# wonheeML/mtl-ssl

Hardware: AMD Instinct MI355X
Metric: images/sec training, Faster R-CNN ResNet-101 + aux heads (higher is better)
Workload: dtype f32; 1 GPU; Faster R-CNN ResNet-101 + window/closeness/edgemask heads + refine, synthetic 1024x600 COCO-shaped (90 classes), per-GPU batch 2 (BASELINE.json configs[1]); global_batch=2, parallelism=dp1, pipeline_config=configs/frcnn_resnet101_coco_mtl.config

## Files before the change

include/mtlssl_hip.h:

```cpp
#ifndef MTLSSL_HIP_H_
#define MTLSSL_HIP_H_

#include <stdint.h>

#ifdef __cplusplus
extern "C" {
#endif

typedef void* mtlssl_stream_t;

#define MTLSSL_OK 0
#define MTLSSL_EINVAL (-1)
#define MTLSSL_ELAUNCH (-2)
#define MTLSSL_ECOMM (-3)

#define MTLSSL_ABI_VERSION 12

const char* mtlssl_last_error(void);
int mtlssl_abi_version(void);

int mtlssl_exp_rn(const double* x, double* y, int64_t n, mtlssl_stream_t stream);

typedef struct {
  int32_t N, H, W, C;
  int32_t K, R, S;
  int32_t OH, OW;
  int32_t stride, dilation;
  int32_t pad_t, pad_l;
  int32_t ldy;
} mtlssl_conv_desc;

#define MTLSSL_EPI_BIAS 1
#define MTLSSL_EPI_RESIDUAL 2
#define MTLSSL_EPI_RELU 4
#define MTLSSL_EPI_TANH 8
#define MTLSSL_EPI_RELU6 16
#define MTLSSL_EPI_MASK 32
#define MTLSSL_EPI_ACCUM 64
#define MTLSSL_EPI_MASK6 128

int64_t mtlssl_conv2d_workspace_bytes(const mtlssl_conv_desc* d, int mode);
int mtlssl_conv2d_fwd(const mtlssl_conv_desc* d, const float* x, const float* w,
                      const float* bias, const float* residual, float* y, int epilogue,
                      void* workspace, mtlssl_stream_t stream);
int mtlssl_conv2d_dgrad(const mtlssl_conv_desc* d, const float* dy, const float* w,
                        const float* residual, const float* mask_ref, float* dx, int epilogue,
                        void* workspace, mtlssl_stream_t stream);
int64_t mtlssl_conv2d_filter_xf_bytes(const mtlssl_conv_desc* d, int mode);
int mtlssl_conv2d_filter_xf_variant(const mtlssl_conv_desc* d, int mode);
int mtlssl_conv2d_transform_filter(const mtlssl_conv_desc* d, int mode, int variant, const float* w, float* filter_xf,
                                   mtlssl_stream_t stream);
int mtlssl_conv2d_transform_filters(int variant, int n, const void* w_ptrs, const void* xf_ptrs, const int64_t* ck,
                                    const int32_t* flip, int64_t max_ck, mtlssl_stream_t stream);
int mtlssl_conv2d_fwd_xf(const mtlssl_conv_desc* d, const float* x, const float* w, const float* bias,
                         const float* residual, float* y, int epilogue, void* workspace, const float* filter_xf,
                         int xf_variant, mtlssl_stream_t stream);
int mtlssl_conv2d_dgrad_xf(const mtlssl_conv_desc* d, const float* dy, const float* w, const float* residual,
                           const float* mask_ref, float* dx, int epilogue, void* workspace, const float* filter_xf,
                           int xf_variant, mtlssl_stream_t stream);
int64_t mtlssl_conv2d_input_xf_bytes(const mtlssl_conv_desc* d, int variant);
int mtlssl_conv2d_fwd_keep(const mtlssl_conv_desc* d, const float* x, const float* w, const float* bias,
                           const float* residual, float* y, int epilogue, void* workspace, const float* filter_xf,
                           int xf_variant, float* input_xf, int input_variant, mtlssl_stream_t stream);
int mtlssl_conv2d_wgrad_xf(const mtlssl_conv_desc* d, const float* x, const float* dy,
                           const float* out_scale, float* dw, float* dbias, float beta,
                           void* workspace, const float* input_xf, int input_variant, mtlssl_stream_t stream);
#define MTLSSL_CONV_GROUP_MAX 4
typedef struct {
  const float* w;
// ... 114 lines not shown
#define MTLSSL_EVAL_NMS_STANDARD 1
#define MTLSSL_EVAL_NMS_SOFT_LINEAR 2
#define MTLSSL_EVAL_NMS_SOFT_GAUSSIAN 3
int mtlssl_eval_nms(const float* boxes, const float* scores, const int32_t* segment_offsets, int num_segments,
                    int max_segment, int nms_type, double iou_threshold, double sigma, double scale_y, double scale_x,
                    int max_output, int32_t* index_out, float* scores_out, int32_t* count_out,
                    mtlssl_stream_t stream);
int mtlssl_edgemask_agreement(const float* logits, int Hf, int Wf, const float* gt_mask, int h, int w,
                              int32_t* count_out, mtlssl_stream_t stream);

#define MTLSSL_AUX_MAX_GT 256
#define MTLSSL_AUX_WINDOW_ATTEMPTS 100
int mtlssl_aux_draw_windows(const float* boxes_norm, const int32_t* num, int batch, int max_gt, int num_windows,
                            double height, double width, double min_obj_size, uint32_t seed, uint32_t step,
                            uint32_t image0, float* window_boxes, mtlssl_stream_t stream);
int mtlssl_aux_window_labels(const float* boxes_norm, const float* classes_bg, const int32_t* num,
                             const float* window_boxes, int batch, int max_gt, int num_classes, int num_windows,
                             double height, double width, float* labels_out, mtlssl_stream_t stream);
int mtlssl_aux_closeness(const float* boxes_norm, const float* classes_bg, const int32_t* num, int batch, int max_gt,
                         int num_classes, double height, double width, float* closeness_out, mtlssl_stream_t stream);
int mtlssl_aux_edgemask(const float* boxes_norm, const int32_t* num, int batch, int max_gt, double height, double width,
                        int mask_size, float* edgemask_out, mtlssl_stream_t stream);

int64_t mtlssl_assign_targets_workspace_bytes(int batch, int n, int max_gt);
int mtlssl_assign_targets(const float* anchors, int anchors_batched, int batch, int n,
                          const float* gt_boxes, const int32_t* num_gt, int max_gt,
                          const float* gt_labels, int label_dim, const float* gt_extra,
                          int extra_dim, const float* unmatched_cls_target, float matched_thresh,
                          float unmatched_thresh, int force_match, int32_t* match_out,
                          float* cls_targets_out, float* cls_weights_out, float* reg_targets_out,
                          float* reg_weights_out, float* extra_targets_out, void* workspace,
                          mtlssl_stream_t stream);

int mtlssl_balanced_sample(const float* indicator, const float* labels, int batch, int n,
                           int batch_size, float positive_fraction, uint32_t seed,
                           uint32_t stream_id0, uint32_t stream_stride, float* sampled_out,
                           mtlssl_stream_t stream);

int mtlssl_sample_proposals(const float* proposals, const int32_t* num_proposals, int batch,
                            int max_p, const float* gt_boxes, const int32_t* num_gt, int max_gt,
                            const float* gt_labels_bg, int label_dim, int n2,
                            float balance_fraction, uint32_t seed, uint32_t stream_id0,
                            uint32_t stream_stride, float img_h, float img_w,
                            float* boxes_abs_out, float* boxes_norm_out, int32_t* num_out,
                            mtlssl_stream_t stream);

int mtlssl_roi_crop_pool_fwd(const float* feat, int B, int H, int W, int C, const float* boxes,
                             const int32_t* box_ind, int R, int crop, int pool_k, int pool_stride,
                             float* out, uint8_t* argmax_out, mtlssl_stream_t stream);
int mtlssl_roi_crop_pool_bwd(const float* dout, const uint8_t* argmax, int B, int H, int W, int C,
                             const float* boxes, const int32_t* box_ind, int R, int crop,
                             int pool_k, int pool_stride, float* dfeat, mtlssl_stream_t stream);
int64_t mtlssl_roi_crop_pool_bwd_workspace_bytes(void);
int mtlssl_roi_crop_pool_bwd_ex(const float* dout, const uint8_t* argmax, int B, int H, int W, int C,
                                const float* boxes, const int32_t* box_ind, int R, int crop, int pool_k,
                                int pool_stride, float* dfeat, int accumulate, int algo, void* workspace,
                                mtlssl_stream_t stream);

int mtlssl_psroi_fwd(const float* fmap, int B, int H, int W, int C, const float* boxes,
                     const int32_t* box_ind, int R, int crop_h, int crop_w, int bins_y, int bins_x,
                     float* out, mtlssl_stream_t stream);
int mtlssl_psroi_bwd(const float* dout, int B, int H, int W, int C, const float* boxes,
                     const int32_t* box_ind, int R, int crop_h, int crop_w, int bins_y, int bins_x,
                     float* dfmap, mtlssl_stream_t stream);

int mtlssl_resize_bilinear_fwd(const float* x, float* y, int N, int H, int W, int C, int OH,
                               int OW, mtlssl_stream_t stream);
int mtlssl_resize_bilinear_bwd(const float* dy, float* dx, int N, int H, int W, int C, int OH,
                               int OW, mtlssl_stream_t stream);

typedef struct {
  int64_t offset;
  int32_t H, W;
  int32_t flip;
  float sy, sx;
  int32_t pad;
} mtlssl_image_desc;
int mtlssl_prepare_images(const uint8_t* pixels, const mtlssl_image_desc* desc, int B, int OH, int OW, float* out,
                          mtlssl_stream_t stream);
int64_t mtlssl_prepare_images_aug_workspace(int B, int n_contrast, int max_H);
int mtlssl_prepare_images_aug(const uint8_t* pixels, const mtlssl_image_desc* desc, int B, int OH, int OW,
                              const int32_t* prog, int n_ops, const float* params, int P, int max_H, void* workspace,
                              int64_t workspace_bytes, float* out, mtlssl_stream_t stream);


int mtlssl_smooth_l1_fwd_bwd(const float* pred, const float* target, const float* row_scale,
                             int rows, int code_size, float sigma, float* row_loss_out,
                             float* dpred_out, mtlssl_stream_t stream);
int mtlssl_softmax_ce_fwd_bwd(const float* logits, int ld_logits, const float* targets,
                              int ld_targets, int col0, int C, const float* row_scale, int rows,
                              float* row_loss_out, float* dlogits_out, mtlssl_stream_t stream);
int mtlssl_reduce_sum(const float* x, int n, float scale, float* out, mtlssl_stream_t stream);

int64_t mtlssl_sgd_workspace_bytes(int num_vars, int64_t max_var_size);
int mtlssl_sgd_momentum_clip(float* weights, const float* grads, float* accum,
                             const int32_t* var_offsets, int num_vars, int64_t total,
                             int64_t max_var_size, float lr, float momentum, float clip_norm,
                             float grad_scale, const float* var_weight_decay, const float* var_grad_mult,
                             float* norms_ws, mtlssl_stream_t stream);
int mtlssl_sgd_momentum_clip_fold(float* weights, float* grads, float* accum,
                                  const int32_t* var_offsets, int num_vars, int64_t total,
                                  int64_t max_var_size, float lr, float momentum, float clip_norm,
                                  float grad_scale, const float* var_weight_decay, const float* var_grad_mult,
                                  float* norms_ws, float* eff, const void* scale_ptrs, const int32_t* scale_len,
                                  int zero_grads, mtlssl_stream_t stream);
int mtlssl_adaptive_update_clip(int kind, float* weights, const float* grads, float* slot0, float* slot1,
// ... 78 lines not shown
```

mtl_ssl_amd/csrc/ops.hip:

```cpp
#include "common.h"

namespace mtlssl {

struct CropGeom {
  float y1, x1, hs, ws;
  int b;
};
__device__ __forceinline__ CropGeom crop_geom(const float* boxes, const int32_t* box_ind, int r,
                                              int H, int W, int crop) {
  float4 bx = *reinterpret_cast<const float4*>(boxes + (int64_t)r * 4);
  CropGeom g;
  g.b = box_ind[r];
  if (crop > 1) {
    g.hs = (bx.z - bx.x) * (float)(H - 1) / (float)(crop - 1);
    g.ws = (bx.w - bx.y) * (float)(W - 1) / (float)(crop - 1);
    g.y1 = bx.x * (float)(H - 1);
    g.x1 = bx.y * (float)(W - 1);
  } else {
    g.hs = 0.f; g.ws = 0.f;
    g.y1 = 0.5f * (bx.x + bx.z) * (float)(H - 1);
    g.x1 = 0.5f * (bx.y + bx.w) * (float)(W - 1);
  }
  return g;
}
// ... 134 lines not shown
    int dy = s / pk, dx = s % pk;
    float in_y = g.y1 + (float)(py * ps + dy) * g.hs;
    float in_x = g.x1 + (float)(px * ps + dx) * g.ws;
    if (in_y < 0.f || in_y > (float)(H - 1) || in_x < 0.f || in_x > (float)(W - 1)) continue;
    int ty = (int)floorf(in_y), by = (int)ceilf(in_y);
    int lx = (int)floorf(in_x), rx = (int)ceilf(in_x);
    float yl = in_y - (float)ty, xl = in_x - (float)lx;
    float dtop = (1.f - yl) * gr, dbot = yl * gr;
    unsafeAtomicAdd(fb + ((int64_t)ty * W + lx) * C + c, (1.f - xl) * dtop);
    unsafeAtomicAdd(fb + ((int64_t)ty * W + rx) * C + c, xl * dtop);
    unsafeAtomicAdd(fb + ((int64_t)by * W + lx) * C + c, (1.f - xl) * dbot);
    unsafeAtomicAdd(fb + ((int64_t)by * W + rx) * C + c, xl * dbot);
  }
}

constexpr int kRoiSlice = 16;
constexpr int kRoiPass = 512;
constexpr int kRoiThreads = 512;
struct RoiItem { float y1, x1, hs, ws; };

__global__ void __launch_bounds__(256) k_absmax_bits(const float* __restrict__ x, int64_t n4, uint32_t* out) {
  uint32_t m = 0;
  const int64_t stride = (int64_t)gridDim.x * 256;
  const uint4* x4 = reinterpret_cast<const uint4*>(x);
  int64_t i = (int64_t)blockIdx.x * 256 + threadIdx.x;
  for (; i + 3 * stride < n4; i += 4 * stride) {
    uint4 a = x4[i], b = x4[i + stride], c = x4[i + 2 * stride], d = x4[i + 3 * stride];
    uint32_t ma = max(max(a.x & 0x7fffffffu, a.y & 0x7fffffffu), max(a.z & 0x7fffffffu, a.w & 0x7fffffffu));
    uint32_t mb = max(max(b.x & 0x7fffffffu, b.y & 0x7fffffffu), max(b.z & 0x7fffffffu, b.w & 0x7fffffffu));
    uint32_t mc = max(max(c.x & 0x7fffffffu, c.y & 0x7fffffffu), max(c.z & 0x7fffffffu, c.w & 0x7fffffffu));
    uint32_t md = max(max(d.x & 0x7fffffffu, d.y & 0x7fffffffu), max(d.z & 0x7fffffffu, d.w & 0x7fffffffu));
    m = max(m, max(max(ma, mb), max(mc, md)));
  }
  for (; i < n4; i += stride) {
    uint4 a = x4[i];
    m = max(m, max(max(a.x & 0x7fffffffu, a.y & 0x7fffffffu), max(a.z & 0x7fffffffu, a.w & 0x7fffffffu)));
  }
#pragma unroll
  for (int o = 32; o > 0; o >>= 1) m = max(m, (uint32_t)__shfl_xor((int)m, o, 64));
  __shared__ uint32_t s_m[4];
  if ((threadIdx.x & 63) == 0) s_m[threadIdx.x >> 6] = m;
  __syncthreads();
  if (threadIdx.x == 0) {
    m = max(max(s_m[0], s_m[1]), max(s_m[2], s_m[3]));
    if (m) atomicMax(out, m);
  }
}

template <int PK>
__global__ void __launch_bounds__(kRoiThreads)
    k_roi_crop_pool_bwd_lds(const float* __restrict__ dout, const uint8_t* __restrict__ argmax, int H,
                            int W, int C, const float* __restrict__ boxes,
                            const int32_t* __restrict__ box_ind, int R, int crop, int pk_rt, int ps, int PH,
                            int PW, int band_rows, int nbands, int accumulate,
                            const uint32_t* __restrict__ absmax_bits, float* __restrict__ dfeat) {
  extern __shared__ __attribute__((aligned(16))) unsigned char s_raw[];
  const int pk = PK ? PK : pk_rt;
  const int NP = band_rows * W;
  unsigned long long* acc = reinterpret_cast<unsigned long long*>(s_raw);
  RoiItem* s_geom = reinterpret_cast<RoiItem*>(acc + (size_t)kRoiSlice * NP);
  int* s_roi = reinterpret_cast<int*>(s_geom + kRoiPass);
  uint16_t* s_entry = reinterpret_cast<uint16_t*>(s_roi + kRoiPass);
  __shared__ int s_n;
  int nblk = gridDim.x, bid = blockIdx.x;
  if (nblk % 8 == 0) bid = (bid % 8) * (nblk / 8) + bid / 8;
  const int band = bid % nbands;
  const int slice = (bid / nbands) % (C / kRoiSlice);
  const int img = bid / nbands / (C / kRoiSlice);
  const int row0 = band * band_rows;
  const int rows = min(band_rows, H - row0);
  const int tid = threadIdx.x;
  const uint32_t mbits = *absmax_bits;
  const bool finite = mbits < 0x7f800000u;
  int e = (int)(mbits >> 23) - 126;
  e = max(e, -90);
  const float scale = __uint_as_float((uint32_t)(30 - e + 127) << 23);
  const double descale = __longlong_as_double((long long)(e - 30 + 1023) << 52);
  for (int i = tid; i < kRoiSlice * NP; i += kRoiThreads) acc[i] = 0ull;
  const int quad = tid & 3;
  const int cslot = tid >> 2;
  unsigned long long* qacc = acc + (size_t)(quad * 4) * NP;
  const float inv_pw = 1.0f / (float)PW;
  const int cells = PH * PW;
  const float Hm1 = (float)(H - 1), Wm1 = (float)(W - 1);
  for (int base = 0; base < R; base += kRoiPass) {
    if (tid == 0) s_n = 0;
    __syncthreads();
    int lim = min(R, base + kRoiPass);
    for (int r = base + tid; r < lim; r += kRoiThreads) {
      if (box_ind[r] != img) continue;
      CropGeom g = crop_geom(boxes, box_ind, r, H, W, crop);
      int lo = PH, hi = -1;
      for (int py = 0; py < PH; ++py) {
        float ya = g.y1 + (float)(py * ps) * g.hs, yb = g.y1 + (float)(py * ps + pk - 1) * g.hs;
        float mn = fminf(ya, yb), mx = fmaxf(ya, yb);
        if (floorf(mn) < (float)(row0 + rows) && ceilf(mx) >= (float)row0) { lo = min(lo, py); hi = max(hi, py); }
      }
      if (hi < lo) continue;
      int slot = r - base;
      s_geom[slot] = RoiItem{g.y1, g.x1, g.hs, g.ws};
      s_roi[slot] = r;
      int pos = atomicAdd(&s_n, hi - lo + 1);
      for (int py = lo; py <= hi; ++py) s_entry[pos + py - lo] = (uint16_t)(slot * 64 + py);
    }
    __syncthreads();
    const int ncell = s_n * PW;
    RoiItem g_n = {0.f, 0.f, 0.f, 0.f};
    float4 gr_n = make_float4(0.f, 0.f, 0.f, 0.f);
    uint32_t am_n = 0u;
    int py_n = 0, px_n = 0;
    bool ok_n = false;
    auto fetch = [&](int ci) {
      ok_n = ci < ncell;
      if (!ok_n) return;
      int ei = (int)(((float)ci + 0.5f) * inv_pw);
      px_n = ci - ei * PW;
      int ent = s_entry[ei];
      int slot = ent >> 6;
      py_n = ent & 63;
      g_n = s_geom[slot];
      int64_t o = ((int64_t)s_roi[slot] * cells + py_n * PW + px_n) * C + slice * kRoiSlice + quad * 4;
      gr_n = *reinterpret_cast<const float4*>(dout + o);
      am_n = argmax ? *reinterpret_cast<const uint32_t*>(argmax + o) : 0u;
    };
    fetch(cslot);
    for (int c0 = 0; c0 < ncell; c0 += kRoiThreads / 4) {
      const RoiItem g = g_n;
      const float4 gr4 = gr_n;
      const uint32_t am4 = am_n;
      const int py = py_n, px = px_n;
      const bool ok = ok_n;
      fetch(c0 + kRoiThreads / 4 + cslot);
      if (!ok) continue;
      float grv[4] = {gr4.x, gr4.y, gr4.z, gr4.w};
      if (PK == 1) {
        float in_y = g.y1 + (float)(py * ps) * g.hs, in_x = g.x1 + (float)(px * ps) * g.ws;
        if (in_y < 0.f || in_y > Hm1 || in_x < 0.f || in_x > Wm1) continue;
        int ty = (int)floorf(in_y), by = (int)ceilf(in_y), lx = (int)floorf(in_x), rx = (int)ceilf(in_x);
        float yl = in_y - (float)ty, xl = in_x - (float)lx;
        int t = ty - row0, b = by - row0;
        bool okt = t >= 0 && t < rows, okb = b >= 0 && b < rows;
// ... 964 lines not shown
    o[e] *= sc[r];
    r = r + 1 == K ? 0 : r + 1;
  }
  *reinterpret_cast<float4*>(eff + i) = make_float4(o[0], o[1], o[2], o[3]);
}
__global__ void k_tanh_bwd(const float* y, const float* dy, float* dx, int64_t n) {
  int64_t i = blockIdx.x * (int64_t)blockDim.x + threadIdx.x;
  if (i < n) dx[i] = dy[i] * (1.f - y[i] * y[i]);
}

}

using namespace mtlssl;

extern "C" {

int mtlssl_roi_crop_pool_fwd(const float* feat, int B, int H, int W, int C, const float* boxes,
                             const int32_t* box_ind, int R, int crop, int pk, int ps, float* out,
                             uint8_t* argmax, mtlssl_stream_t stream) {
  MTLSSL_REQUIRE(C % 4 == 0, "roi_crop: C must be a multiple of 4");
  MTLSSL_REQUIRE(pk >= 1 && ps >= 1 && crop >= pk && pk * pk <= 255, "roi_crop: bad pool geometry");
  if (R == 0) return MTLSSL_OK;
  int PH = (crop - pk) / ps + 1;
  const char* algo = getenv("MTLSSL_ROI_FWD");
  if (C % 32 == 0 && C / 32 <= 256 && pk <= 2 && algo && !strcmp(algo, "xcd")) {
    const char* se = getenv("MTLSSL_ROI_SLICES");
    int nsl = se ? atoi(se) : 8;
    if (nsl != 8 && nsl != 4 && nsl != 2 && nsl != 1) nsl = 8;
    while (nsl < 8 && C / (4 * nsl) > 256) nsl *= 2;
    const int rep = 8 / nsl;
    const int L = C / (4 * nsl), CB = 256 / L;
    const int groups = (int)cdiv(cdiv(PH * PH, CB), rep);
    const dim3 grid(groups * 8, R), block((unsigned)align_up(CB * L, 64));
    if (pk == 1)
      hipLaunchKernelGGL(k_roi_crop_pool_fwd_xcd<1>, grid, block, 0, S(stream), feat, H, W, C, boxes, box_ind, crop, ps, PH, PH,
                         L, CB, rep, out, argmax);
    else
      hipLaunchKernelGGL(k_roi_crop_pool_fwd_xcd<2>, grid, block, 0, S(stream), feat, H, W, C, boxes, box_ind, crop, ps, PH, PH,
                         L, CB, rep, out, argmax);
    return check_launch("roi_crop_pool_fwd");
  }
  int threads = (int)align_up(C / 4 < 256 ? C / 4 : 256, 64);
  hipLaunchKernelGGL(k_roi_crop_pool_fwd, dim3(PH * PH, R), dim3(threads), 0, S(stream), feat, H, W,
                     C, boxes, box_ind, crop, pk, ps, PH, PH, out, argmax);
  return check_launch("roi_crop_pool_fwd");
}
int mtlssl_roi_crop_pool_bwd(const float* dout, const uint8_t* argmax, int B, int H, int W, int C,
                             const float* boxes, const int32_t* box_ind, int R, int crop, int pk,
                             int ps, float* dfeat, mtlssl_stream_t stream) {
  return mtlssl_roi_crop_pool_bwd_ex(dout, argmax, B, H, W, C, boxes, box_ind, R, crop, pk, ps, dfeat, 1, 2, nullptr,
                                     stream);
}

static size_t roi_bwd_lds_bytes(int band_rows, int W, int PH) {
  return sizeof(unsigned long long) * kRoiSlice * (size_t)(band_rows * W) +
         kRoiPass * (sizeof(RoiItem) + sizeof(int) + sizeof(uint16_t) * (size_t)PH);
}

int64_t mtlssl_roi_crop_pool_bwd_workspace_bytes(void) { return 256; }

int mtlssl_roi_crop_pool_bwd_ex(const float* dout, const uint8_t* argmax, int B, int H, int W, int C,
                                const float* boxes, const int32_t* box_ind, int R, int crop, int pk, int ps,
                                float* dfeat, int accumulate, int algo, void* workspace, mtlssl_stream_t stream) {
  MTLSSL_REQUIRE(argmax != nullptr || pk == 1, "roi_crop_bwd: argmax required when pooling");
  MTLSSL_REQUIRE(algo >= 0 && algo <= 2, "roi_crop_bwd: algo must be 0 (auto), 1 (LDS-resident, deterministic) or 2 (HBM atomics)");
  MTLSSL_REQUIRE(pk >= 1 && ps >= 1 && crop >= pk, "roi_crop_bwd: bad pool geometry");
  int PH = (crop - pk) / ps + 1;
  size_t lists = roi_bwd_lds_bytes(0, W, PH);
  int band_rows = lists < 76 * 1024 ? (int)((76 * 1024 - lists) / (sizeof(unsigned long long) * kRoiSlice * (size_t)W)) : 0;
  if (band_rows > H) band_rows = H;
  bool lds_ok = C % kRoiSlice == 0 && band_rows >= 1 && B >= 1 && PH <= 64 && workspace != nullptr;
  MTLSSL_REQUIRE(algo != 1 || lds_ok, "roi_crop_bwd: the LDS-resident kernel needs C %% 16 == 0, a workspace, at most 64 cell rows and a "
                                      "map row that fits its LDS budget (W = %d)", W);
  if (algo == 2 || !lds_ok) {
    if (!accumulate)
      if (hipMemsetAsync(dfeat, 0, sizeof(float) * (size_t)B * H * W * C, S(stream)) != hipSuccess) {
        set_error("roi_crop_pool_bwd: memset failed");
        return MTLSSL_ELAUNCH;
      }
    if (R == 0) return MTLSSL_OK;
    hipLaunchKernelGGL(k_roi_crop_pool_bwd, dim3(PH * PH, R), dim3(256), 0, S(stream), dout, argmax, H,
                       W, C, boxes, box_ind, crop, pk, ps, PH, PH, dfeat);
    return check_launch("roi_crop_pool_bwd");
  }
  if (R == 0 && accumulate) return MTLSSL_OK;
  uint32_t* amax = reinterpret_cast<uint32_t*>(workspace);
  if (hipMemsetAsync(amax, 0, sizeof(uint32_t), S(stream)) != hipSuccess) {
    set_error("roi_crop_pool_bwd: memset failed");
    return MTLSSL_ELAUNCH;
  }
  int64_t n4 = (int64_t)R * PH * PH * C / 4;
  if (n4 > 0)
    hipLaunchKernelGGL(k_absmax_bits, dim3((unsigned)(n4 < 1024 * 256 ? cdiv(n4, 256) : 1024)), dim3(256), 0, S(stream),
                       dout, n4, amax);
  int nbands = (int)cdiv(H, band_rows);
  band_rows = (int)cdiv(H, nbands);
  size_t lds = roi_bwd_lds_bytes(band_rows, W, PH);
  int grid = nbands * (C / kRoiSlice) * B;
  auto kern = pk == 1 ? k_roi_crop_pool_bwd_lds<1> : pk == 2 ? k_roi_crop_pool_bwd_lds<2> : k_roi_crop_pool_bwd_lds<0>;
  if (int rc = ensure_dynamic_lds(reinterpret_cast<const void*>(kern), lds > 96 * 1024 ? lds : 96 * 1024, "roi_crop_pool_bwd_lds")) return rc;
  hipLaunchKernelGGL(kern, dim3(grid), dim3(kRoiThreads), lds, S(stream), dout, argmax, H, W, C, boxes, box_ind, R, crop, pk, ps,
                     PH, PH, band_rows, nbands, accumulate, amax, dfeat);
  return check_launch("roi_crop_pool_bwd_lds");
}

int mtlssl_psroi_fwd(const float* fmap, int B, int H, int W, int C, const float* boxes,
                     const int32_t* box_ind, int R, int crop_h, int crop_w, int bins_y, int bins_x,
                     float* out, mtlssl_stream_t stream) {
  MTLSSL_REQUIRE(bins_y >= 1 && bins_x >= 1, "num_spatial_bins should be >= 1");
  MTLSSL_REQUIRE(crop_h % bins_y == 0 && crop_w % bins_x == 0,
                 "crop_size should be divisible by num_spatial_bins");
  MTLSSL_REQUIRE(C % (bins_y * bins_x) == 0, "depth must be divisible by the number of bins");
  if (R == 0) return MTLSSL_OK;
  int Cc = C / (bins_y * bins_x);
  hipLaunchKernelGGL(k_psroi_fwd, dim3(R), dim3(256), sizeof(float) * Cc * bins_y * bins_x, S(stream), fmap, H, W, C, boxes,
                     box_ind, bins_y, bins_x, crop_h / bins_y, crop_w / bins_x, Cc, out);
  return check_launch("psroi_fwd");
}
int mtlssl_psroi_bwd(const float* dout, int B, int H, int W, int C, const float* boxes,
                     const int32_t* box_ind, int R, int crop_h, int crop_w, int bins_y, int bins_x,
                     float* dfmap, mtlssl_stream_t stream) {
  MTLSSL_REQUIRE(bins_y >= 1 && bins_x >= 1 && crop_h % bins_y == 0 && crop_w % bins_x == 0 &&
                     C % (bins_y * bins_x) == 0, "psroi_bwd: bad geometry");
  if (R == 0) return MTLSSL_OK;
  int Cc = C / (bins_y * bins_x);
  MTLSSL_REQUIRE(C <= 1024 && bins_y <= kPsBins && bins_x <= kPsBins,
                 "psroi_bwd: at most 1024 score-map channels and 8 bins per side");
  const size_t lds = (size_t)kPsChunk * (bins_y + bins_x + 1) * 4 + (size_t)kPsChunk * bins_y * bins_x * 2;
  if (int rc = ensure_dynamic_lds(reinterpret_cast<const void*>(k_psroi_bwd_gather), lds, "psroi_bwd")) return rc;
  hipLaunchKernelGGL(k_psroi_bwd_gather, dim3((unsigned)(B * H * W)), dim3(256), lds, S(stream),
                     dout, H, W, C, boxes, box_ind, R, bins_y, bins_x, crop_h / bins_y, crop_w / bins_x, Cc, dfmap);
  return check_launch("psroi_bwd");
}

int mtlssl_resize_bilinear_fwd(const float* x, float* y, int N, int H, int W, int C, int OH, int OW,
                               mtlssl_stream_t stream) {
  int64_t total = (int64_t)N * OH * OW * C;
  if (!total) return MTLSSL_OK;
  hipLaunchKernelGGL(k_resize_fwd, dim3(cdiv(total, 256)), dim3(256), 0, S(stream), x, y, H, W, C,
                     OH, OW, (float)H / (float)OH, (float)W / (float)OW, total);
  return check_launch("resize_fwd");
}
int mtlssl_prepare_images(const uint8_t* pixels, const mtlssl_image_desc* desc, int B, int OH, int OW, float* out,
                          mtlssl_stream_t stream) {
  MTLSSL_REQUIRE(B >= 0 && B <= 65535 && OH > 0 && OW > 0, "prepare_images: bad geometry");
  if (!B) return MTLSSL_OK;
  const int64_t pix = (int64_t)OH * OW;
  hipLaunchKernelGGL(k_prepare_images, dim3((unsigned)cdiv(pix, 256), (unsigned)B), dim3(256), 0, S(stream), pixels,
                     desc, OH, OW, out);
  return check_launch("prepare_images");
}
int64_t mtlssl_prepare_images_aug_workspace(int B, int n_contrast, int max_H) {
  if (B <= 0 || n_contrast <= 0) return 0;
  const int64_t means = ((int64_t)B * n_contrast * 3 * 4 + 255) / 256 * 256;
  return means + (int64_t)B * max_H * 3 * 8;
}
int mtlssl_prepare_images_aug(const uint8_t* pixels, const mtlssl_image_desc* desc, int B, int OH, int OW,
                              const int32_t* prog, int n_ops, const float* params, int P, int max_H, void* workspace,
                              int64_t workspace_bytes, float* out, mtlssl_stream_t stream) {
  MTLSSL_REQUIRE(B >= 0 && B <= 65535 && OH > 0 && OW > 0, "prepare_images_aug: bad geometry");
  MTLSSL_REQUIRE(n_ops >= 0 && n_ops <= kAugMaxOps, "prepare_images_aug: %d ops, at most %d", n_ops, kAugMaxOps);
  MTLSSL_REQUIRE(n_ops == 0 || prog, "prepare_images_aug: null program");
  AugProgram pr;
  pr.n = n_ops;
  int need = 0, n_contrast = 0;
  for (int i = 0; i < n_ops; ++i) {
    MTLSSL_REQUIRE(prog[i] >= 0 && prog[i] < kAugNumOps, "prepare_images_aug: bad op code %d at op %d", prog[i], i);
// ... 274 lines not shown
```

mtl_ssl_amd/csrc/winograd.hip:

```cpp
#include "conv_mfma.h"
#include "conv_split.h"

namespace mtlssl {

namespace {

struct F43 {
  static constexpr int P = 6, I = 6, O = 4;
  static constexpr float bt(int a, int i) {
    constexpr float t[6][6] = {{4, 0, -5, 0, 1, 0}, {0, -4, -4, 1, 1, 0}, {0, 4, -4, -1, 1, 0},
                               {0, -2, -1, 2, 1, 0}, {0, 2, -1, -2, 1, 0}, {0, 4, 0, -5, 0, 1}};
    return t[a][i];
  }
  static constexpr float at(int u, int a) {
    constexpr float t[4][6] = {{1, 1, 1, 1, 1, 0}, {0, 1, -1, 2, -2, 0}, {0, 1, 1, 4, 4, 0}, {0, 1, -1, 8, -8, 1}};
    return t[u][a];
  }
  static constexpr float g(int a, int r) {
    constexpr float t[6][3] = {{1.f / 4, 0, 0}, {-1.f / 6, -1.f / 6, -1.f / 6}, {-1.f / 6, 1.f / 6, -1.f / 6},
                               {1.f / 24, 1.f / 12, 1.f / 6}, {1.f / 24, -1.f / 12, 1.f / 6}, {0, 0, 1}};
    return t[a][r];
  }
};
struct F33 {
// ... 77 lines not shown
}
__device__ __forceinline__ floatx4 act_fwd(floatx4 v, int epi) {
#pragma unroll
  for (int q = 0; q < 4; ++q) v[q] = act_fwd(v[q], epi);
  return v;
}
__device__ __forceinline__ float mask_bwd(float g, float y, int epi) { return act_mask(g, y, epi); }
__device__ __forceinline__ floatx4 mask_bwd(floatx4 g, floatx4 y, int epi) {
#pragma unroll
  for (int q = 0; q < 4; ++q) g[q] = act_mask(g[q], y[q], epi);
  return g;
}

template <typename S, typename VT>
__device__ __forceinline__ void wino_filter_one(const float* w, float* U, int64_t CK, int flip, int64_t i) {
  constexpr int P = S::P;
  VT t[P][3];
#pragma unroll
  for (int s = 0; s < 3; ++s) {
    VT col[3], o[P];
#pragma unroll
    for (int r = 0; r < 3; ++r) {
      int rr = flip ? 2 - r : r, ss = flip ? 2 - s : s;
      col[r] = *reinterpret_cast<const VT*>(w + (int64_t)(rr * 3 + ss) * CK + i);
    }
    xform<S, XF_G, P, 3>(col, o);
#pragma unroll
    for (int a = 0; a < P; ++a) t[a][s] = o[a];
  }
#pragma unroll
  for (int a = 0; a < P; ++a) {
    VT o[P];
    xform<S, XF_G, P, 3>(t[a], o);
#pragma unroll
    for (int b = 0; b < P; ++b) *reinterpret_cast<VT*>(U + (int64_t)(a * P + b) * CK + i) = o[b];
  }
}
template <typename S, typename VT>
__global__ void __launch_bounds__(256) k_wino_filter(const float* w, float* U, int64_t CK, int flip) {
  int64_t i = (blockIdx.x * (int64_t)256 + threadIdx.x) * (sizeof(VT) / 4);
  if (i >= CK) return;
  wino_filter_one<S, VT>(w, U, CK, flip, i);
}
template <typename S>
__global__ void __launch_bounds__(256) k_wino_filter_batched(const float* const* w, float* const* U, const int64_t* CK,
                                                             const int32_t* flip) {
  const int l = blockIdx.y;
  const int64_t ck = CK[l];
  int64_t i = blockIdx.x * (int64_t)256 + threadIdx.x;
  if (i >= ck) return;
  wino_filter_one<S, float>(w[l], U[l], ck, flip[l], i);
}

template <typename S, typename VT>
__global__ void __launch_bounds__(256) k_wino_input(const float* in, float* V, WinoGeom g, int C, int ld) {
  constexpr int P = S::P, I = S::I;
  const TileIdx ix = tile_index<VT>(g, C);
  if (!ix.ok) return;
  const int y0 = S::O * ix.ty - 1, x0 = S::O * ix.tx - 1;
  const float* base = in + ((int64_t)ix.n * g.H * g.W) * ld + ix.c;
  VT tmp[P][I];
#pragma unroll
  for (int j = 0; j < I; ++j) {
    const int x = x0 + j;
    const bool okx = (unsigned)x < (unsigned)g.W;
    VT col[I], o[P];
#pragma unroll
    for (int i = 0; i < I; ++i) {
      const int y = y0 + i;
      const bool ok = okx && (unsigned)y < (unsigned)g.H;
      col[i] = ok ? *reinterpret_cast<const VT*>(base + ((int64_t)y * g.W + x) * ld) : VT{};
    }
    xform<S, XF_BT, P, I>(col, o);
#pragma unroll
    for (int a = 0; a < P; ++a) tmp[a][j] = o[a];
  }
  const int64_t plane = g.T * C;
  float* vp = V + ix.t * C + ix.c;
#pragma unroll
  for (int a = 0; a < P; ++a) {
    VT o[P];
    xform<S, XF_BT, P, I>(tmp[a], o);
#pragma unroll
    for (int b = 0; b < P; ++b) *reinterpret_cast<VT*>(vp + (int64_t)(a * P + b) * plane) = o[b];
  }
}

template <typename S, typename VT>
__global__ void __launch_bounds__(256) k_wino_dy(const float* dy, float* dM, WinoGeom g, int K, int ld) {
  constexpr int P = S::P, O = S::O;
  const TileIdx ix = tile_index<VT>(g, K);
  if (!ix.ok) return;
  const float* base = dy + ((int64_t)ix.n * g.H * g.W) * ld + ix.c;
  VT tmp[P][O];
#pragma unroll
  for (int j = 0; j < O; ++j) {
    const int x = O * ix.tx + j;
    VT col[O], o[P];
#pragma unroll
    for (int i = 0; i < O; ++i) {
      const int y = O * ix.ty + i;
      const bool ok = y < g.H && x < g.W;
      col[i] = ok ? *reinterpret_cast<const VT*>(base + ((int64_t)y * g.W + x) * ld) : VT{};
    }
    xform<S, XF_A, P, O>(col, o);
#pragma unroll
    for (int a = 0; a < P; ++a) tmp[a][j] = o[a];
  }
  const int64_t plane = g.T * K;
  float* mp = dM + ix.t * K + ix.c;
#pragma unroll
  for (int a = 0; a < P; ++a) {
    VT o[P];
    xform<S, XF_A, P, O>(tmp[a], o);
#pragma unroll
    for (int b = 0; b < P; ++b) *reinterpret_cast<VT*>(mp + (int64_t)(a * P + b) * plane) = o[b];
  }
}

template <typename S, int MODE, typename VT>
__global__ void __launch_bounds__(256) k_wino_output(const float* Mb, float* out, WinoGeom g, int K, int ldo,
                                                     const float* bias, const float* residual,
                                                     const float* mask, int epi) {
  constexpr int P = S::P, O = S::O;
  const TileIdx ix = tile_index<VT>(g, K);
  if (!ix.ok) return;
  const int64_t plane = g.T * K;
  const float* mp = Mb + ix.t * K + ix.c;
  VT tmp[O][P];
#pragma unroll
  for (int b = 0; b < P; ++b) {
    VT col[P], o[O];
#pragma unroll
    for (int a = 0; a < P; ++a) col[a] = *reinterpret_cast<const VT*>(mp + (int64_t)(a * P + b) * plane);
    xform<S, XF_AT, O, P>(col, o);
#pragma unroll
    for (int u = 0; u < O; ++u) tmp[u][b] = o[u];
  }
  VT bv{};
  if constexpr (MODE == MODE_FWD)
    if (epi & MTLSSL_EPI_BIAS) bv = *reinterpret_cast<const VT*>(bias + ix.c);
#pragma unroll
  for (int u = 0; u < O; ++u) {
    VT o[O];
    xform<S, XF_AT, O, P>(tmp[u], o);
    const int oy = O * ix.ty + u;
    if (oy >= g.H) continue;
#pragma unroll
    for (int v_ = 0; v_ < O; ++v_) {
      const int ox = O * ix.tx + v_;
      if (ox >= g.W) continue;
      const int64_t pix = ((int64_t)ix.n * g.H + oy) * g.W + ox;
      const int64_t off = pix * K + ix.c;
      const int64_t offo = pix * ldo + ix.c;
      VT v = o[v_];
      if constexpr (MODE == MODE_FWD) {
        v += bv;
        if (epi & MTLSSL_EPI_RESIDUAL) v += *reinterpret_cast<const VT*>(residual + off);
        v = act_fwd(v, epi);
      } else {
        if (epi & MTLSSL_EPI_RESIDUAL) v += *reinterpret_cast<const VT*>(residual + off);
        if (epi & MTLSSL_EPI_ACCUM) v += *reinterpret_cast<const VT*>(out + offo);
        if (epi & MASK_ANY) v = mask_bwd(v, *reinterpret_cast<const VT*>(mask + off), epi);
      }
      *reinterpret_cast<VT*>(out + offo) = v;
    }
  }
}

template <typename S, typename VT>
__global__ void __launch_bounds__(256) k_wino_wgrad_out(const float* dU, int nsplit, int64_t CK, int K,
                                                        const float* scale, float* dw, float beta) {
  constexpr int P = S::P;
  int64_t i = (blockIdx.x * (int64_t)256 + threadIdx.x) * (sizeof(VT) / 4);
  if (i >= CK) return;
  VT u[P][P];
#pragma unroll
  for (int a = 0; a < P; ++a)
#pragma unroll
    for (int b = 0; b < P; ++b) u[a][b] = *reinterpret_cast<const VT*>(dU + (int64_t)(a * P + b) * CK + i);
  for (int z = 1; z < nsplit; ++z) {
#pragma unroll
    for (int a = 0; a < P; ++a)
#pragma unroll
      for (int b = 0; b < P; ++b)
        u[a][b] += *reinterpret_cast<const VT*>(dU + ((int64_t)z * (P * P) + a * P + b) * CK + i);
  }
  VT t[3][P];
#pragma unroll
  for (int b = 0; b < P; ++b) {
    VT col[P], o[3];
#pragma unroll
    for (int a = 0; a < P; ++a) col[a] = u[a][b];
    xform<S, XF_GT, 3, P>(col, o);
#pragma unroll
    for (int r = 0; r < 3; ++r) t[r][b] = o[r];
  }
  VT sc{};
  if (scale) sc = *reinterpret_cast<const VT*>(scale + i % K);
#pragma unroll
  for (int r = 0; r < 3; ++r) {
    VT o[3];
    xform<S, XF_GT, 3, P>(t[r], o);
#pragma unroll
    for (int s = 0; s < 3; ++s) {
      VT v = scale ? o[s] * sc : o[s];
      VT* p = reinterpret_cast<VT*>(dw + (int64_t)(r * 3 + s) * CK + i);
      *p = beta != 0.f ? beta * *p + v : v;
    }
  }
}

typedef float floatx2 __attribute__((ext_vector_type(2)));

template <typename S>
WinoGeom geom(const mtlssl_conv_desc* d) {
  WinoGeom g;
  g.N = d->N; g.H = d->H; g.W = d->W;
  g.th = (int)cdiv(d->H, S::O); g.tw = (int)cdiv(d->W, S::O);
  g.T = (int64_t)d->N * g.th * g.tw;
  return g;
}

template <typename S> constexpr bool can_vec() { return S::P <= 6; }
// ... 293 lines not shown
```

mtl_ssl_amd/lib.py:

```python
import ctypes
import os
import re

HERE = os.path.dirname(os.path.abspath(__file__))
HEADER = os.path.join(HERE, "..", "include", "mtlssl_hip.h")
LIB_PATH = os.environ.get("MTLSSL_LIB_PATH") or os.path.join(HERE, "libmtlssl_hip.so")


class ConvDesc(ctypes.Structure):
    _fields_ = [(n, ctypes.c_int32) for n in
                ("N", "H", "W", "C", "K", "R", "S", "OH", "OW", "stride", "dilation",
                 "pad_t", "pad_l", "ldy")]


_SCALARS = {
    "int": ctypes.c_int, "int32_t": ctypes.c_int32, "int64_t": ctypes.c_int64,
    "uint32_t": ctypes.c_uint32, "float": ctypes.c_float, "double": ctypes.c_double,
    "mtlssl_stream_t": ctypes.c_void_p, "mtlssl_comm_t": ctypes.c_void_p,
}


def _ctype(decl):
    decl = decl.strip()
    if "*" in decl:
        if "mtlssl_conv_desc" in decl:
            return ctypes.POINTER(ConvDesc)
        return ctypes.c_void_p
    base = decl.replace("const", "").split()
    return _SCALARS[base[0]]


def parse_header(path=HEADER):
    text = open(path).read()
    text = re.sub(r"/\*.*?\*/", "", text, flags=re.S)
    protos = {}
    for m in re.finditer(r"\b(int|int64_t|const char\*)\s+(mtlssl_\w+)\s*\(([^)]*)\)\s*;", text):
        ret, name, args = m.group(1), m.group(2), m.group(3)
        restype = {"int": ctypes.c_int, "int64_t": ctypes.c_int64,
                   "const char*": ctypes.c_char_p}[ret]
        argtypes = []
        if args.strip() not in ("", "void"):
            for a in args.split(","):
                a = a.strip()
                a = re.sub(r"\s*\w+$", "", a) if not a.endswith("*") else a
                argtypes.append(_ctype(a))
        protos[name] = (restype, argtypes)
    return protos


class MtlsslError(RuntimeError):
    pass


class _Lib:
    def __init__(self):
        if not os.path.exists(LIB_PATH):
            raise MtlsslError(
                "%s not found: build it with `python -m mtl_ssl_amd.build` "
                "(there is no CPU fallback for the product path)" % LIB_PATH)
        import torch
        self.cdll = ctypes.CDLL(LIB_PATH)
        self.protos = parse_header()
        want = int(re.search(r"#define\s+MTLSSL_ABI_VERSION\s+(\d+)", open(HEADER).read()).group(1))
        self.cdll.mtlssl_abi_version.restype = ctypes.c_int
        have = self.cdll.mtlssl_abi_version()
        if have != want:
            raise MtlsslError("%s has ABI version %d, include/mtlssl_hip.h declares %d: rebuild it with "
                              "`python -m mtl_ssl_amd.build`" % (LIB_PATH, have, want))
        for name, (restype, argtypes) in self.protos.items():
            fn = getattr(self.cdll, name)
            fn.restype = restype
            fn.argtypes = argtypes
            if restype is ctypes.c_int and name not in ("mtlssl_abi_version", "mtlssl_conv2d_tile_config", "mtlssl_conv2d_num_dispatches",
                                                        "mtlssl_conv2d_set_winograd", "mtlssl_conv2d_set_fp32_engine", "mtlssl_conv2d_filter_xf_variant",
                                                        "mtlssl_conv2d_set_pointwise"):
                setattr(self, name[len("mtlssl_"):], self._checked(fn, name))
            else:
                setattr(self, name[len("mtlssl_"):], fn)

    def _checked(self, fn, name):
        last_error = self.cdll.mtlssl_last_error

        def call(*args):
            rc = fn(*args)
            if rc != 0:
                raise MtlsslError("%s failed (%d): %s" % (name, rc, last_error().decode()))
        return call


_lib = None


def lib():
    global _lib
    if _lib is None:
        _lib = _Lib()
    return _lib


def ptr(t):
    return None if t is None else t.data_ptr()
```

mtl_ssl_amd/ops.py:

```python
import ctypes
import os

import numpy as np
import torch

from .lib import ConvDesc, lib, ptr

EPI_BIAS, EPI_RESIDUAL, EPI_RELU, EPI_TANH, EPI_RELU6, EPI_MASK, EPI_ACCUM, EPI_MASK6 = 1, 2, 4, 8, 16, 32, 64, 128
f32 = torch.float32
i32 = torch.int32


_raw_stream = getattr(torch._C, "_cuda_getCurrentRawStream", None)
_cur_device = getattr(torch._C, "_cuda_getDevice", None)


def _stream():
    if _raw_stream is not None and _cur_device is not None:
        return _raw_stream(_cur_device())
    return torch.cuda.current_stream().cuda_stream


def _chk(t, dtype=f32):
    assert t.is_cuda and t.is_contiguous() and t.dtype == dtype, (t.device, t.dtype, t.is_contiguous())
# ... 1000 lines not shown
    B, n = indicator.shape
    out = torch.empty_like(indicator)
    lib().balanced_sample(ptr(_chk(indicator)), ptr(_chk(labels)), B, n, batch_size,
                          float(positive_fraction), seed, stream_id0, stream_stride, ptr(out),
                          _stream())
    return out


def sample_proposals(proposals, num_proposals, gt_boxes, num_gt, gt_labels_bg, n2,
                     balance_fraction, seed, stream_id0, stream_stride, img_h, img_w):
    B, max_p, _ = proposals.shape
    dev = proposals.device
    G, d = gt_labels_bg.shape[1], gt_labels_bg.shape[2]
    ob = torch.empty((B, n2, 4), dtype=f32, device=dev)
    on = torch.empty((B, n2, 4), dtype=f32, device=dev)
    num = torch.empty((B,), dtype=i32, device=dev)
    lib().sample_proposals(ptr(_chk(proposals)), ptr(_chk(num_proposals, i32)), B, max_p,
                           ptr(_chk(gt_boxes)), ptr(_chk(num_gt, i32)), G, ptr(_chk(gt_labels_bg)),
                           d, n2, float(balance_fraction), seed, stream_id0, stream_stride,
                           float(img_h), float(img_w), ptr(ob), ptr(on), ptr(num), _stream())
    return ob, on, num


def roi_crop_pool_fwd(feat, boxes, box_ind, crop, pool_k=1, pool_stride=1, want_argmax=True):
    B, H, W, C = feat.shape
    R = boxes.shape[0]
    P = (crop - pool_k) // pool_stride + 1
    out = torch.empty((R, P, P, C), dtype=f32, device=feat.device)
    am = (torch.empty((R, P, P, C), dtype=torch.uint8, device=feat.device)
          if (want_argmax and pool_k > 1) else None)
    t0 = _hbm_begin("roi_crop_pool_fwd")
    lib().roi_crop_pool_fwd(ptr(_chk(feat)), B, H, W, C, ptr(_chk(boxes)), ptr(_chk(box_ind, i32)),
                            R, crop, pool_k, pool_stride, ptr(out), ptr(am), _stream())
    if t0 is not None:
        HBM_PROFILER.end("roi_crop_pool_fwd", 4 * (feat.numel() + out.numel()) + (am.numel() if am is not None else 0), t0)
    return out, am


def roi_crop_pool_bwd(dout, argmax, feat_shape, boxes, box_ind, crop, pool_k, pool_stride,
                      dfeat=None, accumulate=None, algo=0):
    B, H, W, C = feat_shape
    if dfeat is None:
        dfeat = torch.empty(feat_shape, dtype=f32, device=dout.device)
        accumulate = False
    elif accumulate is None:
        accumulate = True
    ws = workspace(lib().roi_crop_pool_bwd_workspace_bytes(), "roi_bwd", dout.device)
    lib().roi_crop_pool_bwd_ex(ptr(_chk(dout)), ptr(argmax), B, H, W, C, ptr(boxes), ptr(box_ind),
                               boxes.shape[0], crop, pool_k, pool_stride, ptr(dfeat), 1 if accumulate else 0,
                               int(algo), ptr(ws), _stream())
    return dfeat


def psroi_fwd(fmap, boxes, box_ind, crop, bins):
    B, H, W, C = fmap.shape
    R = boxes.shape[0]
    Cc = C // max(bins[0] * bins[1], 1)
    out = torch.empty((R, Cc), dtype=f32, device=fmap.device)
    t0 = _hbm_begin("psroi_fwd")
    lib().psroi_fwd(ptr(_chk(fmap)), B, H, W, C, ptr(_chk(boxes)), ptr(_chk(box_ind, i32)), R, crop[0],
                    crop[1], bins[0], bins[1], ptr(out), _stream())
    if t0 is not None:
        HBM_PROFILER.end("psroi_fwd", 4 * (fmap.numel() + out.numel()), t0)
    return out


def psroi_bwd(dout, fmap_shape, boxes, box_ind, crop, bins, dfmap=None):
    B, H, W, C = fmap_shape
    if dfmap is None:
        dfmap = torch.zeros(fmap_shape, dtype=f32, device=dout.device)
    t0 = _hbm_begin("psroi_bwd")
    lib().psroi_bwd(ptr(_chk(dout)), B, H, W, C, ptr(_chk(boxes)), ptr(_chk(box_ind, i32)), boxes.shape[0],
                    crop[0], crop[1], bins[0], bins[1], ptr(dfmap), _stream())
    if t0 is not None:
        HBM_PROFILER.end("psroi_bwd", 4 * (dout.numel() + dfmap.numel()), t0)
    return dfmap


def resize_bilinear_fwd(x, OH, OW):
    N, H, W, C = x.shape
    y = torch.empty((N, OH, OW, C), dtype=f32, device=x.device)
    lib().resize_bilinear_fwd(ptr(_chk(x)), ptr(y), N, H, W, C, OH, OW, _stream())
    return y


IMAGE_DESC = np.dtype({"names": ["offset", "H", "W", "flip", "sy", "sx", "pad"],
                       "formats": ["<i8", "<i4", "<i4", "<i4", "<f4", "<f4", "<i4"],
                       "offsets": [0, 8, 12, 16, 20, 24, 28], "itemsize": 32})


def image_descs(shapes, flips, OH, OW):
    d = np.zeros(len(shapes), IMAGE_DESC)
    off = 0
    for i, ((H, W), f) in enumerate(zip(shapes, flips)):
        assert H >= 1 and W >= 1, (H, W)
        d[i] = (off, H, W, int(bool(f)), np.float32(H / OH), np.float32(W / OW), 0)
        off += int(H) * int(W) * 3
    return d, off


def prepare_images(pixels, desc, B, OH, OW, out=None):
    assert pixels.is_cuda and pixels.dtype == torch.uint8 and desc.is_cuda and desc.dtype == torch.uint8
    assert desc.numel() >= B * IMAGE_DESC.itemsize and desc.data_ptr() % 8 == 0
    if out is None:
        out = torch.empty((B, OH, OW, 3), dtype=f32, device=pixels.device)
    assert tuple(out.shape) == (B, OH, OW, 3)
# ... 224 lines not shown
```

Before: 37.15 images/sec.

## Shrink ROI crop-pool backward LDS budget and raise Winograd transform occupancy

The LDS-resident ROI crop-pool backward kernel now plans its band height and ROI pass size from a configurable LDS budget, 32 KiB by default instead of about 76 KiB. Smaller blocks let several workgroups share a CU and increase the number of bands, at the cost of more blocks each rescanning the ROI list. Separately, the Winograd output and weight-gradient transforms for large tiles get a minimum-waves launch bound to cap register use and raise occupancy, which risks spills. A psroi LDS size check and a query API for band counts are also added.

```diff
diff --git a/include/mtlssl_hip.h b/include/mtlssl_hip.h
--- a/include/mtlssl_hip.h
+++ b/include/mtlssl_hip.h
@@ -14,7 +14,7 @@
 #define MTLSSL_ELAUNCH (-2)
 #define MTLSSL_ECOMM (-3)
 
-#define MTLSSL_ABI_VERSION 12
+#define MTLSSL_ABI_VERSION 13
 
 const char* mtlssl_last_error(void);
 int mtlssl_abi_version(void);
@@ -235,6 +235,7 @@
                              const float* boxes, const int32_t* box_ind, int R, int crop,
                              int pool_k, int pool_stride, float* dfeat, mtlssl_stream_t stream);
 int64_t mtlssl_roi_crop_pool_bwd_workspace_bytes(void);
+int mtlssl_roi_crop_pool_bwd_bands(int H, int W, int crop, int pool_k, int pool_stride, int algo);
 int mtlssl_roi_crop_pool_bwd_ex(const float* dout, const uint8_t* argmax, int B, int H, int W, int C,
                                 const float* boxes, const int32_t* box_ind, int R, int crop, int pool_k,
                                 int pool_stride, float* dfeat, int accumulate, int algo, void* workspace,
diff --git a/mtl_ssl_amd/csrc/ops.hip b/mtl_ssl_amd/csrc/ops.hip
--- a/mtl_ssl_amd/csrc/ops.hip
+++ b/mtl_ssl_amd/csrc/ops.hip
@@ -210,15 +210,15 @@
     k_roi_crop_pool_bwd_lds(const float* __restrict__ dout, const uint8_t* __restrict__ argmax, int H,
                             int W, int C, const float* __restrict__ boxes,
                             const int32_t* __restrict__ box_ind, int R, int crop, int pk_rt, int ps, int PH,
-                            int PW, int band_rows, int nbands, int accumulate,
+                            int PW, int band_rows, int nbands, int pass, int accumulate,
                             const uint32_t* __restrict__ absmax_bits, float* __restrict__ dfeat) {
   extern __shared__ __attribute__((aligned(16))) unsigned char s_raw[];
   const int pk = PK ? PK : pk_rt;
   const int NP = band_rows * W;
   unsigned long long* acc = reinterpret_cast<unsigned long long*>(s_raw);
   RoiItem* s_geom = reinterpret_cast<RoiItem*>(acc + (size_t)kRoiSlice * NP);
-  int* s_roi = reinterpret_cast<int*>(s_geom + kRoiPass);
-  uint16_t* s_entry = reinterpret_cast<uint16_t*>(s_roi + kRoiPass);
+  int* s_roi = reinterpret_cast<int*>(s_geom + pass);
+  uint16_t* s_entry = reinterpret_cast<uint16_t*>(s_roi + pass);
   __shared__ int s_n;
   int nblk = gridDim.x, bid = blockIdx.x;
   if (nblk % 8 == 0) bid = (bid % 8) * (nblk / 8) + bid / 8;
@@ -241,10 +241,10 @@
   const float inv_pw = 1.0f / (float)PW;
   const int cells = PH * PW;
   const float Hm1 = (float)(H - 1), Wm1 = (float)(W - 1);
-  for (int base = 0; base < R; base += kRoiPass) {
+  for (int base = 0; base < R; base += pass) {
     if (tid == 0) s_n = 0;
     __syncthreads();
-    int lim = min(R, base + kRoiPass);
+    int lim = min(R, base + pass);
     for (int r = base + tid; r < lim; r += kRoiThreads) {
       if (box_ind[r] != img) continue;
       CropGeom g = crop_geom(boxes, box_ind, r, H, W, crop);
@@ -1315,9 +1315,38 @@
                                      stream);
 }
 
-static size_t roi_bwd_lds_bytes(int band_rows, int W, int PH) {
+static size_t roi_bwd_lds_bytes(int band_rows, int W, int PH, int pass) {
   return sizeof(unsigned long long) * kRoiSlice * (size_t)(band_rows * W) +
-         kRoiPass * (sizeof(RoiItem) + sizeof(int) + sizeof(uint16_t) * (size_t)PH);
+         pass * (sizeof(RoiItem) + sizeof(int) + sizeof(uint16_t) * (size_t)PH);
+}
+
+constexpr int kRoiLdsKiBMax = 76;
+#ifndef MTLSSL_ROI_BWD_LDS_KIB
+#define MTLSSL_ROI_BWD_LDS_KIB 32
+#endif
+constexpr int kRoiLdsKiBDefault = MTLSSL_ROI_BWD_LDS_KIB;
+
+struct RoiBwdPlan { int band_rows, nbands, pass; size_t lds; };
+static RoiBwdPlan roi_bwd_plan(int H, int W, int PH, int kib) {
+  if (kib <= 0) {
+    RoiBwdPlan d = roi_bwd_plan(H, W, PH, kRoiLdsKiBDefault);
+    return d.band_rows >= 1 ? d : roi_bwd_plan(H, W, PH, kRoiLdsKiBMax);
+  }
+  if (kib > kRoiLdsKiBMax) kib = kRoiLdsKiBMax;
+  RoiBwdPlan p;
+  p.pass = kib >= 64 ? kRoiPass : kib >= 40 ? kRoiPass / 2 : kRoiPass / 4;
+  const size_t budget = (size_t)kib * 1024, lists = roi_bwd_lds_bytes(0, W, PH, p.pass);
+  p.band_rows = lists < budget ? (int)((budget - lists) / (sizeof(unsigned long long) * kRoiSlice * (size_t)W)) : 0;
+  if (p.band_rows > H) p.band_rows = H;
+  p.nbands = p.band_rows >= 1 ? (int)cdiv(H, p.band_rows) : 0;
+  if (p.nbands) p.band_rows = (int)cdiv(H, p.nbands);
+  p.lds = roi_bwd_lds_bytes(p.band_rows, W, PH, p.pass);
+  return p;
+}
+
+int mtlssl_roi_crop_pool_bwd_bands(int H, int W, int crop, int pk, int ps, int algo) {
+  if (pk < 1 || ps < 1 || crop < pk || H < 1 || W < 1 || algo < 0 || (algo & 0xff) > 2 || (algo >> 16)) return 0;
+  return roi_bwd_plan(H, W, (crop - pk) / ps + 1, algo >> 8).nbands;
 }
 
 int64_t mtlssl_roi_crop_pool_bwd_workspace_bytes(void) { return 256; }
@@ -1326,15 +1355,16 @@
                                 const float* boxes, const int32_t* box_ind, int R, int crop, int pk, int ps,
                                 float* dfeat, int accumulate, int algo, void* workspace, mtlssl_stream_t stream) {
   MTLSSL_REQUIRE(argmax != nullptr || pk == 1, "roi_crop_bwd: argmax required when pooling");
-  MTLSSL_REQUIRE(algo >= 0 && algo <= 2, "roi_crop_bwd: algo must be 0 (auto), 1 (LDS-resident, deterministic) or 2 (HBM atomics)");
+  MTLSSL_REQUIRE(algo >= 0 && (algo & 0xff) <= 2 && (algo >> 16) == 0,
+                 "roi_crop_bwd: algo must be 0 (auto), 1 (LDS-resident, deterministic) or 2 (HBM atomics), + 256 * the LDS budget in KiB");
+  const int lds_kib = algo >> 8;
+  algo &= 0xff;
   MTLSSL_REQUIRE(pk >= 1 && ps >= 1 && crop >= pk, "roi_crop_bwd: bad pool geometry");
   int PH = (crop - pk) / ps + 1;
-  size_t lists = roi_bwd_lds_bytes(0, W, PH);
-  int band_rows = lists < 76 * 1024 ? (int)((76 * 1024 - lists) / (sizeof(unsigned long long) * kRoiSlice * (size_t)W)) : 0;
-  if (band_rows > H) band_rows = H;
-  bool lds_ok = C % kRoiSlice == 0 && band_rows >= 1 && B >= 1 && PH <= 64 && workspace != nullptr;
+  const RoiBwdPlan plan = roi_bwd_plan(H, W, PH, lds_kib);
+  bool lds_ok = C % kRoiSlice == 0 && plan.band_rows >= 1 && B >= 1 && PH <= 64 && workspace != nullptr;
   MTLSSL_REQUIRE(algo != 1 || lds_ok, "roi_crop_bwd: the LDS-resident kernel needs C %% 16 == 0, a workspace, at most 64 cell rows and a "
-                                      "map row that fits its LDS budget (W = %d)", W);
+                                      "map row that fits its LDS budget (W = %d, %d KiB)", W, lds_kib ? lds_kib : kRoiLdsKiBDefault);
   if (algo == 2 || !lds_ok) {
     if (!accumulate)
       if (hipMemsetAsync(dfeat, 0, sizeof(float) * (size_t)B * H * W * C, S(stream)) != hipSuccess) {
@@ -1356,14 +1386,11 @@
   if (n4 > 0)
     hipLaunchKernelGGL(k_absmax_bits, dim3((unsigned)(n4 < 1024 * 256 ? cdiv(n4, 256) : 1024)), dim3(256), 0, S(stream),
                        dout, n4, amax);
-  int nbands = (int)cdiv(H, band_rows);
-  band_rows = (int)cdiv(H, nbands);
-  size_t lds = roi_bwd_lds_bytes(band_rows, W, PH);
-  int grid = nbands * (C / kRoiSlice) * B;
+  int grid = plan.nbands * (C / kRoiSlice) * B;
   auto kern = pk == 1 ? k_roi_crop_pool_bwd_lds<1> : pk == 2 ? k_roi_crop_pool_bwd_lds<2> : k_roi_crop_pool_bwd_lds<0>;
-  if (int rc = ensure_dynamic_lds(reinterpret_cast<const void*>(kern), lds > 96 * 1024 ? lds : 96 * 1024, "roi_crop_pool_bwd_lds")) return rc;
-  hipLaunchKernelGGL(kern, dim3(grid), dim3(kRoiThreads), lds, S(stream), dout, argmax, H, W, C, boxes, box_ind, R, crop, pk, ps,
-                     PH, PH, band_rows, nbands, accumulate, amax, dfeat);
+  if (int rc = ensure_dynamic_lds(reinterpret_cast<const void*>(kern), 96 * 1024, "roi_crop_pool_bwd_lds")) return rc;
+  hipLaunchKernelGGL(kern, dim3(grid), dim3(kRoiThreads), plan.lds, S(stream), dout, argmax, H, W, C, boxes, box_ind, R, crop, pk, ps,
+                     PH, PH, plan.band_rows, plan.nbands, plan.pass, accumulate, amax, dfeat);
   return check_launch("roi_crop_pool_bwd_lds");
 }
 
@@ -1376,6 +1403,8 @@
   MTLSSL_REQUIRE(C % (bins_y * bins_x) == 0, "depth must be divisible by the number of bins");
   if (R == 0) return MTLSSL_OK;
   int Cc = C / (bins_y * bins_x);
+  MTLSSL_REQUIRE((size_t)C * sizeof(float) <= 64 * 1024,
+                 "psroi_fwd: one partial per (bin, channel) is kept in LDS: at most 16384 score-map channels (C = %d)", C);
   hipLaunchKernelGGL(k_psroi_fwd, dim3(R), dim3(256), sizeof(float) * Cc * bins_y * bins_x, S(stream), fmap, H, W, C, boxes,
                      box_ind, bins_y, bins_x, crop_h / bins_y, crop_w / bins_x, Cc, out);
   return check_launch("psroi_fwd");
diff --git a/mtl_ssl_amd/csrc/winograd.hip b/mtl_ssl_amd/csrc/winograd.hip
--- a/mtl_ssl_amd/csrc/winograd.hip
+++ b/mtl_ssl_amd/csrc/winograd.hip
@@ -153,6 +153,11 @@
   wino_filter_one<S, float>(w[l], U[l], ck, flip[l], i);
 }
 
+#ifndef MTLSSL_M7_XF_WAVES
+#define MTLSSL_M7_XF_WAVES 4
+#endif
+template <typename S> constexpr int xf_min_waves(int mode) { return (S::P > 6 && mode != MODE_FWD) ? MTLSSL_M7_XF_WAVES : 1; }
+
 template <typename S, typename VT>
 __global__ void __launch_bounds__(256) k_wino_input(const float* in, float* V, WinoGeom g, int C, int ld) {
   constexpr int P = S::P, I = S::I;
@@ -220,7 +225,7 @@
 }
 
 template <typename S, int MODE, typename VT>
-__global__ void __launch_bounds__(256) k_wino_output(const float* Mb, float* out, WinoGeom g, int K, int ldo,
+__global__ void __launch_bounds__(256, xf_min_waves<S>(MODE)) k_wino_output(const float* Mb, float* out, WinoGeom g, int K, int ldo,
                                                      const float* bias, const float* residual,
                                                      const float* mask, int epi) {
   constexpr int P = S::P, O = S::O;
@@ -270,7 +275,7 @@
 }
 
 template <typename S, typename VT>
-__global__ void __launch_bounds__(256) k_wino_wgrad_out(const float* dU, int nsplit, int64_t CK, int K,
+__global__ void __launch_bounds__(256, xf_min_waves<S>(MODE_WGRAD)) k_wino_wgrad_out(const float* dU, int nsplit, int64_t CK, int K,
                                                         const float* scale, float* dw, float beta) {
   constexpr int P = S::P;
   int64_t i = (blockIdx.x * (int64_t)256 + threadIdx.x) * (sizeof(VT) / 4);
diff --git a/mtl_ssl_amd/lib.py b/mtl_ssl_amd/lib.py
--- a/mtl_ssl_amd/lib.py
+++ b/mtl_ssl_amd/lib.py
@@ -73,7 +73,7 @@
             fn.argtypes = argtypes
             if restype is ctypes.c_int and name not in ("mtlssl_abi_version", "mtlssl_conv2d_tile_config", "mtlssl_conv2d_num_dispatches",
                                                         "mtlssl_conv2d_set_winograd", "mtlssl_conv2d_set_fp32_engine", "mtlssl_conv2d_filter_xf_variant",
-                                                        "mtlssl_conv2d_set_pointwise"):
+                                                        "mtlssl_conv2d_set_pointwise", "mtlssl_roi_crop_pool_bwd_bands"):
                 setattr(self, name[len("mtlssl_"):], self._checked(fn, name))
             else:
                 setattr(self, name[len("mtlssl_"):], fn)
diff --git a/mtl_ssl_amd/ops.py b/mtl_ssl_amd/ops.py
--- a/mtl_ssl_amd/ops.py
+++ b/mtl_ssl_amd/ops.py
@@ -1076,6 +1076,17 @@
     return dfeat
 
 
+ROI_BWD_LDS_KIB = (32, 48, 76)
+
+
+def roi_bwd_algo(algo, lds_kib=0):
+    return int(algo) | (int(lds_kib) << 8)
+
+
+def roi_crop_pool_bwd_bands(feat_shape, crop, pool_k, pool_stride, algo=0):
+    return lib().roi_crop_pool_bwd_bands(feat_shape[1], feat_shape[2], crop, pool_k, pool_stride, int(algo))
+
+
 def psroi_fwd(fmap, boxes, box_ind, crop, bins):
     B, H, W, C = fmap.shape
     R = boxes.shape[0]
```

Result: no change. 37.11 images/sec (-0.1%).
